# PhiFEM/phiFEM

Measured on NVIDIA B200. Metric: phi-FEM cells assembled/s (tags+CSR), higher is better.
Workload: dtype f64

## Files before the change

### include/phifem_b200.h

```cpp
#ifndef PHIFEM_B200_H
#define PHIFEM_B200_H

#include <stdint.h>

#ifdef __cplusplus
extern "C" {
#endif

#define PHIFEM_B200_ABI_VERSION 1

typedef enum phifem_status {
  PHIFEM_OK = 0,
  PHIFEM_ERR_ARGUMENT = -1,
  PHIFEM_ERR_CUDA = -2,
  PHIFEM_ERR_UNSUPPORTED = -3
} phifem_status;

typedef enum phifem_cell_type {
  PHIFEM_TRIANGLE = 0,
  PHIFEM_QUADRILATERAL = 1,
  PHIFEM_TETRAHEDRON = 2
} phifem_cell_type;

typedef struct phifem_mesh {
// ... 108 lines not shown
  const int16_t* seg_start;
  const int32_t* seg_dest;
  int64_t n_cell_inst;
  const int32_t* cell_verts;
  const int16_t* cell_pos;
  int64_t n_ghost_inst;
  const int32_t* ghost_facet;
  const int16_t* ghost_pos;
  int64_t n_bnd_inst;
  const int32_t* bnd_entity;
  const int16_t* bnd_pos;
} phifem_blocked_plan;

int phifem_assemble_blocked_p1(const phifem_mesh* mesh, const double* phi, const double* f, double sigma,
                               const phifem_blocked_plan* plan, double* data, double* b, void* stream);

typedef struct phifem_row_list {
  int64_t n_listed;
  const int32_t* rows;
  const uint8_t* diag_pos;
  const int32_t* ptr;
  const uint32_t* rec;
} phifem_row_list;

typedef struct phifem_cell_tiles {
  int32_t rows_per_tile;
  int32_t n_tiles;
  int64_t n_listed;
  const int32_t* rows;
  const uint8_t* diag_pos;
  const int32_t* chunk_ptr;
  const int32_t* slot_verts;
  const int32_t* rec_base;
  const uint16_t* rec_off;
  const uint32_t* rec;
  const uint32_t* push;
} phifem_cell_tiles;

typedef struct phifem_rows_plan {
  const int32_t* indptr;
  const int32_t* indices;
  int32_t max_row_nnz;
  int32_t reserved;
  phifem_row_list cells;
  phifem_row_list surface;
  int64_t n_ghost_facets;
  const int32_t* ghost_macro;
  int64_t n_entities;
  const int32_t* entity_macro;
  double* surface_work;
  const double* cell_geom;
  const phifem_cell_tiles* tiles;
  double* surface_static;
} phifem_rows_plan;

int phifem_assemble_rows_p1(const phifem_mesh* mesh, const double* phi, const double* f, double sigma,
                            const phifem_rows_plan* plan, double* data, double* b, void* stream);

typedef struct phifem_pk_space {
  int32_t degree;
  int32_t n_dofs_per_cell;
  int64_t n_dofs;
  const int32_t* dofmap;
} phifem_pk_space;

typedef struct phifem_quadrature {
  int32_t n_cell_points;
  int32_t n_facet_points;
  const double* cell_points;
  const double* cell_weights;
  const double* facet_points;
  const double* facet_weights;
} phifem_quadrature;

int phifem_assemble_cells_pk(const phifem_mesh* mesh, const phifem_pk_space* space_w,
                             const phifem_pk_space* space_phi, const phifem_quadrature* quad,
                             const double* phi, const double* f, const int8_t* cell_tags8,
                             const int32_t* active, int64_t n_active, const int32_t* slots, double sigma,
                             double* data, double* b, void* stream);

int phifem_assemble_boundary_pk(const phifem_mesh* mesh, const phifem_pk_space* space_w,
                                const phifem_pk_space* space_phi, const phifem_quadrature* quad,
                                const double* phi, const int32_t* entities, int64_t n_entities,
                                const int32_t* slots, double* data, void* stream);

int phifem_assemble_ghost_pk(const phifem_mesh* mesh, const phifem_pk_space* space_w,
                             const phifem_pk_space* space_phi, const phifem_quadrature* quad,
                             const double* phi, const int32_t* facets, int64_t n_facets,
                             const int32_t* slots, double sigma, double* data, void* stream);

int phifem_assemble_weak_cells_pk(const phifem_mesh* mesh, const phifem_pk_space* space_w,
                                  const phifem_pk_space* space_phi, const phifem_quadrature* quad,
                                  const double* phi, const double* f, const double* u_d,
                                  const int8_t* cell_tags8, const int32_t* active, int64_t n_active,
                                  const int32_t* slots, const int32_t* mixed_dofmap, double gamma,
                                  double sigma, double* data, double* b, void* stream);

int phifem_assemble_weak_boundary_pk(const phifem_mesh* mesh, const phifem_pk_space* space_w,
                                     const phifem_quadrature* quad, const int32_t* entities,
                                     int64_t n_entities, const int32_t* slots, double* data, void* stream);

int phifem_assemble_weak_ghost_pk(const phifem_mesh* mesh, const phifem_pk_space* space_w,
                                  const phifem_quadrature* quad, const int32_t* facets, int64_t n_facets,
                                  const int32_t* slots, double sigma, double* data, void* stream);

int phifem_csr_spmv(int64_t n_rows, const int32_t* indptr, const int32_t* indices, const double* data,
// ... 114 lines not shown
```

### phifem_b200/_lib.py

```python
import ctypes
import os

import torch

_HERE = os.path.dirname(os.path.abspath(__file__))
LIB_PATH = os.environ.get("PHIFEM_B200_LIB") or os.path.join(_HERE, "libphifem_b200.so")

CELL_TYPE_ID = {"triangle": 0, "quadrilateral": 1, "tetrahedron": 2}
N_COUNTERS = 16
CNT_INTERIOR, CNT_CUT, CNT_EXTERIOR, CNT_UNTAGGED, CNT_ZERO_DEN, CNT_ZERO_DEN_AMBIGUOUS = 0, 1, 2, 3, 4, 5
CNT_FACET_ZERO_DEN, CNT_FACET_CONFLICT, CNT_BOUNDARY_OWNERS = 11, 12, 13
CNT_CALLER0, CNT_CALLER1 = 14, 15

_vp = ctypes.c_void_p


class CMesh(ctypes.Structure):
    _fields_ = [("cell_type", ctypes.c_int32), ("gdim", ctypes.c_int32),
                ("n_vertices", ctypes.c_int64), ("n_cells", ctypes.c_int64),
                ("n_facets", ctypes.c_int64),
                ("x", _vp), ("cells", _vp), ("c2f", _vp), ("f2c", _vp),
                ("detj_min", ctypes.c_double), ("detj_max", ctypes.c_double),
                ("boundary_facets", _vp), ("n_boundary_facets", ctypes.c_int64),
                ("boundary_owner", _vp), ("boundary_scale", _vp), ("x4", _vp)]


class CLevelset(ctypes.Structure):
    _fields_ = [("mode", ctypes.c_int32), ("n_dofs_per_cell", ctypes.c_int32),
                ("n_cell_points", ctypes.c_int32), ("n_facet_points", ctypes.c_int32),
                ("coeffs", _vp), ("dofmap", _vp), ("cell_table", _vp), ("facet_table", _vp),
                ("cell_values", _vp), ("facet_values", _vp), ("coord_grad", _vp)]


class CBlockedPlan(ctypes.Structure):
    _fields_ = [("n_blocks", ctypes.c_int32), ("capacity", ctypes.c_int32),
                ("max_segments", ctypes.c_int32), ("reserved", ctypes.c_int32),
                ("block_desc", _vp), ("seg_start", _vp), ("seg_dest", _vp),
                ("n_cell_inst", ctypes.c_int64), ("cell_verts", _vp), ("cell_pos", _vp),
                ("n_ghost_inst", ctypes.c_int64), ("ghost_facet", _vp), ("ghost_pos", _vp),
                ("n_bnd_inst", ctypes.c_int64), ("bnd_entity", _vp), ("bnd_pos", _vp)]


class CRowList(ctypes.Structure):
    _fields_ = [("n_listed", ctypes.c_int64), ("rows", _vp), ("diag_pos", _vp), ("ptr", _vp), ("rec", _vp)]


class CCellTiles(ctypes.Structure):
    _fields_ = [("rows_per_tile", ctypes.c_int32), ("n_tiles", ctypes.c_int32), ("n_listed", ctypes.c_int64),
                ("rows", _vp), ("diag_pos", _vp), ("chunk_ptr", _vp), ("slot_verts", _vp), ("rec_base", _vp),
                ("rec_off", _vp), ("rec", _vp), ("push", _vp)]


class CRowsPlan(ctypes.Structure):
    _fields_ = [("indptr", _vp), ("indices", _vp), ("max_row_nnz", ctypes.c_int32),
                ("reserved", ctypes.c_int32), ("cells", CRowList), ("surface", CRowList),
                ("n_ghost_facets", ctypes.c_int64), ("ghost_macro", _vp), ("n_entities", ctypes.c_int64),
                ("entity_macro", _vp), ("surface_work", _vp), ("cell_geom", _vp),
                ("tiles", ctypes.POINTER(CCellTiles)), ("surface_static", _vp)]


class CRowsPlanInfo(ctypes.Structure):
    _fields_ = [("n_rows", ctypes.c_int64), ("nnz", ctypes.c_int64), ("n_active", ctypes.c_int64),
                ("n_ghost", ctypes.c_int64), ("n_entities", ctypes.c_int64), ("active", _vp), ("ghost", _vp),
                ("n_cell_records", ctypes.c_int64), ("n_surface_records", ctypes.c_int64),
                ("cells_record_slots", ctypes.c_int64), ("surface_record_slots", ctypes.c_int64)]


class CPkSpace(ctypes.Structure):
    _fields_ = [("degree", ctypes.c_int32), ("n_dofs_per_cell", ctypes.c_int32), ("n_dofs", ctypes.c_int64),
                ("dofmap", _vp)]


class CQuadrature(ctypes.Structure):
    _fields_ = [("n_cell_points", ctypes.c_int32), ("n_facet_points", ctypes.c_int32),
                ("cell_points", _vp), ("cell_weights", _vp), ("facet_points", _vp), ("facet_weights", _vp)]


class CPatternView(ctypes.Structure):
    _fields_ = [("n_rows", ctypes.c_int64), ("nnz", ctypes.c_int64), ("n_active", ctypes.c_int64),
                ("n_ghost", ctypes.c_int64), ("n_entities", ctypes.c_int64), ("indptr", _vp), ("indices", _vp),
                ("active", _vp), ("ghost", _vp), ("slots_cells", _vp), ("slots_ghost", _vp), ("slots_boundary", _vp)]


class CElasticityParams(ctypes.Structure):
    _fields_ = [(n, ctypes.c_double) for n in ("lmbda_in", "mu_in", "lmbda_out", "mu_out", "coef_in", "coef_out",
                                               "gamma", "sigma_s")]


_PK_HEAD = [ctypes.POINTER(CMesh), ctypes.POINTER(CPkSpace), ctypes.POINTER(CPkSpace),
            ctypes.POINTER(CQuadrature)]

_SIGNATURES = {
    "phifem_last_error": (ctypes.c_char_p, []),
    "phifem_abi_version": (ctypes.c_int, []),
    "phifem_post_to_host": (ctypes.c_int, [_vp, _vp, ctypes.c_int32, _vp]),
    "phifem_tags_match": (ctypes.c_int, [_vp, _vp, ctypes.c_int64, _vp, _vp, ctypes.c_int64, _vp, _vp]),
    "phifem_cell_points": (ctypes.c_int, [ctypes.POINTER(CMesh), _vp, ctypes.c_int32, _vp, _vp]),
    "phifem_tag_cells": (ctypes.c_int, [ctypes.POINTER(CMesh), ctypes.POINTER(CLevelset),
                                        ctypes.c_int32, _vp, _vp, _vp, _vp, _vp]),
    "phifem_tag_facets": (ctypes.c_int, [ctypes.POINTER(CMesh), ctypes.POINTER(CLevelset), _vp, _vp,
                                         _vp, _vp, _vp]),
    "phifem_boundary_records": (ctypes.c_int, [ctypes.POINTER(CMesh), _vp, _vp, _vp]),
    "phifem_tag_facets_phase": (ctypes.c_int, [ctypes.POINTER(CMesh), ctypes.POINTER(CLevelset), _vp, _vp,
                                               _vp, _vp, ctypes.c_int32, _vp]),
    "phifem_entity_records": (ctypes.c_int, [ctypes.POINTER(CMesh), _vp, _vp, ctypes.c_int32,
                                             ctypes.c_uint32, _vp, ctypes.c_int64, _vp, _vp]),
    "phifem_assemble_cells_p1": (ctypes.c_int, [ctypes.POINTER(CMesh), _vp, _vp, _vp, _vp,
                                                ctypes.c_int64, _vp, ctypes.c_double, _vp, _vp, _vp]),
    "phifem_assemble_boundary_p1": (ctypes.c_int, [ctypes.POINTER(CMesh), _vp, _vp, ctypes.c_int64,
                                                   _vp, _vp, _vp]),
    "phifem_assemble_ghost_p1": (ctypes.c_int, [ctypes.POINTER(CMesh), _vp, _vp, ctypes.c_int64, _vp,
# ... 156 lines not shown
```

### phifem_b200/assemble.py

```python
import numpy as np
import torch

from . import _lib
from .fem import Function
from .mesh import Measure


class CSRMatrix:

    def __init__(self, indptr, indices, data, shape):
        self.indptr, self.indices, self.data, self.shape = indptr, indices, data, shape

    def to_scipy(self):
        import scipy.sparse as sp
        return sp.csr_matrix((self.data.cpu().numpy(), self.indices.cpu().numpy(),
                              self.indptr.cpu().numpy()), shape=self.shape)


def ghost_macro_vertices(mesh, facets):
    g = facets.long()
    nv = mesh.cells.shape[1]
    out = []
    for side in (0, 1):
        c = mesh.f2c[g, side].long()
        cv = mesh.cells[c].long()
        lf = (mesh.c2f[c].long() == g[:, None]).long().argmax(dim=1)
        if side == 0:
            keep = torch.arange(nv, device=g.device)[None, :] != lf[:, None]
            out.append(cv[keep].reshape(-1, nv - 1))
        out.append(cv.gather(1, lf[:, None]))
    return torch.cat(out, dim=1)


class AssemblyPlan:

    def __init__(self, mesh, cell_tags8, facet_tags8, entities, method="rows", capacity=None,
                 order="auto", row_mask=None, geometry=False, cell_pass="rows", rows_per_tile=256, symbolic="auto"):
        if mesh.cell_type not in ("triangle", "tetrahedron"):
            raise NotImplementedError("P1 assembly supports triangles and tetrahedra")
        dev = mesh.device
        self.mesh = mesh
        self.cell_tags8 = cell_tags8
        self._sig_cells = cell_tags8.clone()
        self._sig_facets = _facet_classes(facet_tags8)
        n = mesh.num_vertices
        nv = mesh.cells.shape[1]
        self.n_rows = n
        ents2 = entities.reshape(-1, 2)
        if ents2.shape[0]:
            t = cell_tags8[ents2[:, 0].long()]
            if not bool(((t == 1) | (t == 2)).all()):
                raise ValueError("a (cell, local facet) entity names a cell that is not tagged 1 or 2: the strong-/weak-"
                                 "Dirichlet plans take the entities of ds(100) (Gamma_h seen from Omega_h)")
        if symbolic not in ("auto", "torch", "native"):
            raise ValueError("symbolic must be 'auto', 'torch' or 'native'")
        native_ok = (method == "rows" and cell_pass == "rows" and not geometry and dev.type == "cuda")
        if symbolic == "native" and not native_ok:
            raise ValueError("the native symbolic phase builds row-gather plans (method='rows', cell_pass='rows') on "
                             "CUDA meshes")
        self._slots = None
        if native_ok and symbolic in ("auto", "native"):
            from . import rows as rows_mod
            try:
                if order == "auto":
                    order = "natural"
                rp = rows_mod.NativeRowsPlan(mesh, cell_tags8, facet_tags8, entities, order=order, row_mask=row_mask)
            except NotImplementedError:
                if symbolic == "native":
                    raise
                rp = None
            if rp is not None:
                self.entities = entities.reshape(-1, 2).to(torch.int32).contiguous()
                self.active, self.ghost, self.indptr, self.indices, self.nnz = rp.active, rp.ghost, rp.indptr, \
                    rp.indices, rp.nnz
                self.blocked, self.rowsplan, self.method, self.symbolic = None, rp, "rows", "native"
                return
        self.symbolic = "torch"
        self.active = torch.nonzero((cell_tags8 == 1) | (cell_tags8 == 2)).reshape(-1).to(torch.int32)
        interior = mesh.f2c[:, 1] >= 0
        self.ghost = torch.nonzero(((facet_tags8 == 2) | (facet_tags8 == 3)) & interior) \
            .reshape(-1).to(torch.int32)
        self.entities = entities.reshape(-1, 2).to(torch.int32).contiguous()

        def pair_keys(dm):
            return (dm[:, :, None] * n + dm[:, None, :]).reshape(dm.shape[0], dm.shape[1] * dm.shape[1])

        dm = mesh.cells[self.active.long()].long()
        keys_c = pair_keys(dm)
        mac = ghost_macro_vertices(mesh, self.ghost)
        keys_g = pair_keys(mac)
        n_c = keys_c.numel()
        uniq, inv = torch.unique(torch.cat([keys_c.reshape(-1), keys_g.reshape(-1)]), sorted=True,
                                 return_inverse=True)
        del keys_c, keys_g
        slots_cells = inv[:n_c].reshape(-1, nv * nv).to(torch.int32).contiguous()
        slots_ghost = inv[n_c:].reshape(-1, (nv + 1) ** 2).to(torch.int32).contiguous()
        del inv
        keys_b = pair_keys(mesh.cells[self.entities[:, 0].long()].long())
        slots_boundary = torch.searchsorted(uniq, keys_b.reshape(-1)).reshape(-1, nv * nv) \
            .to(torch.int32).contiguous()
        self._slots = (slots_cells, slots_ghost, slots_boundary)
        rows = uniq // n
        self.indices = (uniq - rows * n).to(torch.int32).contiguous()
        counts = torch.bincount(rows, minlength=n)
        self.indptr = torch.zeros(n + 1, dtype=torch.int64, device=dev)
        self.indptr[1:] = torch.cumsum(counts, dim=0)
        self.indptr = self.indptr.to(torch.int32).contiguous()
        self.nnz = int(uniq.numel())
        if self.nnz >= 2 ** 31:
            raise NotImplementedError("CSR pattern with %d entries: indptr / slot maps are int32 (PETSc's default "
                                      "index width too); shard the mesh (phifem_b200/partition.py)" % self.nnz)
        self.blocked, self.rowsplan, self.method = None, None, "atomic"
        if method == "rows" and self.nnz > 0:
            from . import rows as rows_mod
            try:
                self.rowsplan = rows_mod.RowsPlan(self, order=order, row_mask=row_mask, geometry=geometry,
                                                  cell_pass=cell_pass, rows_per_tile=rows_per_tile)
                self.method = "rows"
            except NotImplementedError:
                self.rowsplan = None
        elif method == "blocked" and self.active.numel() > 0:
            from . import blocked
            try:
                self.blocked = blocked.BlockedPlan(self, capacity or blocked.DEFAULT_CAPACITY)
                self.method = "blocked"
            except NotImplementedError:
                self.blocked = None
        elif method not in ("rows", "blocked", "atomic"):
            raise ValueError("method must be 'rows', 'blocked' or 'atomic'")

    def _slot_maps(self):
        if self._slots is None:
            n, nv = self.n_rows, self.mesh.cells.shape[1]
            ip = self.indptr.long()
            rows = torch.repeat_interleave(torch.arange(n, device=self.mesh.device), ip[1:] - ip[:-1])
            keys = rows * n + self.indices.long()
            del rows

            def slots(dm):
                k = (dm[:, :, None] * n + dm[:, None, :]).reshape(-1)
                return torch.searchsorted(keys, k).reshape(dm.shape[0], -1).to(torch.int32).contiguous()
            cells = self.mesh.cells
            self._slots = (slots(cells[self.active.long()].long()), slots(ghost_macro_vertices(self.mesh, self.ghost)),
                           slots(cells[self.entities[:, 0].long()].long()))
        return self._slots

    slots_cells = property(lambda self: self._slot_maps()[0])
    slots_ghost = property(lambda self: self._slot_maps()[1])
    slots_boundary = property(lambda self: self._slot_maps()[2])

    def new_outputs(self):
        dev = self.mesh.device
        return (torch.zeros(self.nnz, dtype=torch.float64, device=dev),
                torch.zeros(self.n_rows, dtype=torch.float64, device=dev))

    def matches(self, cells_tags, facets_tags):
        c8, f8, _ = _plan_inputs(self.mesh, cells_tags, facets_tags, None)
        if c8.numel() != self._sig_cells.numel() or f8.numel() != self._sig_facets.numel():
            return False
        if c8.is_cuda:
            bad = torch.empty(1, dtype=torch.int64, device=c8.device)
            _lib.check(_lib.load().phifem_tags_match(_lib.ptr(c8), _lib.ptr(self._sig_cells), c8.numel(), _lib.ptr(f8),
                                                     _lib.ptr(self._sig_facets), f8.numel(), _lib.ptr(bad), _lib.stream()))
            return int(bad.item()) == 0
        return bool(torch.equal(c8, self._sig_cells)) and bool(torch.equal(_facet_classes(f8), self._sig_facets))


def _facet_classes(facet_tags8):
    return ((facet_tags8 == 2) | (facet_tags8 == 3)).to(torch.int8) + 2 * (facet_tags8 == 4).to(torch.int8)


def _plan_inputs(mesh, cells_tags, facets_tags, ds):
    from .mesh_scripts import _narrow_tags
    c8 = getattr(cells_tags, "tags8", None)
    c8 = c8 if c8 is not None else _narrow_tags(cells_tags.values_dev)
    f8 = getattr(facets_tags, "tags8", None)
    f8 = f8 if f8 is not None else _narrow_tags(facets_tags.values_dev)
    if ds is None:
        ents = torch.zeros(0, dtype=torch.int32, device=mesh.device)
    elif isinstance(ds, Measure) and ds.subdomain_data is None:
        bf = mesh.boundary_facets.long()
        owner = mesh.f2c[bf, 0].long()
        lf = (mesh.c2f[owner].long() == bf[:, None]).long().argmax(dim=1)
        ents = torch.stack([owner, lf], dim=1).reshape(-1).to(torch.int32)
    elif hasattr(ds, "integration_entities_dev"):
        ents = ds.integration_entities_dev
    elif torch.is_tensor(ds):
        ents = ds.to(mesh.device)
    else:
        ents = torch.as_tensor(np.asarray(ds, dtype=np.int32), device=mesh.device)
    return c8.contiguous(), f8.contiguous(), ents


def build_plan(mesh, cells_tags, facets_tags, ds=None, method="rows", capacity=None, order="auto",
               V=None, V_phi=None, geometry=False, cell_pass="rows", rows_per_tile=256, symbolic="auto"):
    c8, f8, ents = _plan_inputs(mesh, cells_tags, facets_tags, ds)
    if mesh.cell_type == "quadrilateral":
        if method not in ("rows", "pk"):
            raise ValueError("method=%r: quadrilateral meshes are assembled by the quadrature kernels only" % method)
        if geometry or cell_pass != "rows" or symbolic == "native":
            raise ValueError("geometry, cell_pass and symbolic='native' are options of the row-gather plans, which "
                             "have no quadrilateral implementation")
        from . import fem
        from .assemble_pk import PkAssemblyPlan
        V = fem.functionspace(mesh, 1) if V is None else V
        V_phi = V if V_phi is None else V_phi
        return PkAssemblyPlan(mesh, c8, f8, ents, V, V_phi)
    V_phi = V if V_phi is None else V_phi
    V = V_phi if V is None else V
    if V is not None and (V.degree != 1 or V_phi.degree != 1 or method == "pk"):
        from .assemble_pk import PkAssemblyPlan
        return PkAssemblyPlan(mesh, c8, f8, ents, V, V_phi)
    return AssemblyPlan(mesh, c8, f8, ents, method=method, capacity=capacity,
                        order=order, geometry=geometry, cell_pass=cell_pass, rows_per_tile=rows_per_tile,
                        symbolic=symbolic)


def _device_vector(mesh, v, space=None):
    if isinstance(v, Function):
        if space is None and v.function_space.degree != 1:
            raise NotImplementedError("this plan was built for P1 (vertex dofs); pass V / V_phi to build_plan")
        if space is not None and v.function_space.degree != space.degree:
            raise ValueError("coefficient of degree %d given where the plan expects degree %d"
                             % (v.function_space.degree, space.degree))
        v = v.x.array
    t = v if torch.is_tensor(v) else torch.from_numpy(np.ascontiguousarray(v, dtype=np.float64))
    t = t.to(mesh.device, dtype=torch.float64, non_blocking=True).contiguous()
    n = mesh.num_vertices if space is None else space.num_dofs
    if t.numel() != n:
        raise ValueError("expected %d dof values, got %d" % (n, t.numel()))
    return t


def assemble_into(plan, phi, f, sigma, data, b, marks=None):
    if getattr(plan, "V", None) is not None:
        from .assemble_pk import assemble_pk_into
        return assemble_pk_into(plan, phi, f, sigma, data, b, marks=marks)
    marks_given = marks is not None
    marks = marks or (lambda: None)
    _lib.require_cuda(plan.mesh)
    if getattr(plan, "rowsplan", None) is not None:
        from . import rows as rows_mod
        marks()
        if marks_given:
            rows_mod.assemble_rows_into(plan.rowsplan, phi, f, sigma, data, b, passes=("cells",))
            marks()
            marks()
            rows_mod.assemble_rows_into(plan.rowsplan, phi, f, sigma, data, b, passes=("surface",))
            marks()
        else:
            rows_mod.assemble_rows_into(plan.rowsplan, phi, f, sigma, data, b)
        return data, b
    if getattr(plan, "blocked", None) is not None:
        from . import blocked
        marks()
        blocked.assemble_blocked_into(plan.blocked, phi, f, sigma, data, b)
        marks()
        marks()
        marks()
        return data, b
    lib = _lib.load()
    cm = _lib.c_mesh(plan.mesh)
    st = _lib.stream()
    data.zero_()
    b.zero_()
    marks()
    _lib.check(lib.phifem_assemble_cells_p1(
        cm, _lib.ptr(phi), _lib.ptr(f), _lib.ptr(plan.cell_tags8), _lib.ptr(plan.active),
# ... 75 lines not shown
```

### phifem_b200/csrc/assemble_rows.cu

```cuda
#include <stdlib.h>

#include <type_traits>

#include "common.cuh"
#include "p1_forms.cuh"

namespace phifem {
namespace {

#ifndef PHIFEM_ROWS_BLOCK
#define PHIFEM_ROWS_BLOCK 64
#endif
constexpr int kRowsBlock = PHIFEM_ROWS_BLOCK;
#ifndef PHIFEM_ROWS_MINBLOCKS
#define PHIFEM_ROWS_MINBLOCKS (512 / PHIFEM_ROWS_BLOCK)
#endif
#ifndef PHIFEM_SURF_MINBLOCKS
#define PHIFEM_SURF_MINBLOCKS PHIFEM_ROWS_MINBLOCKS
#endif
#ifndef PHIFEM_SURF_DEPTH
#define PHIFEM_SURF_DEPTH 2
#endif
#ifndef PHIFEM_ONCE_MINBLOCKS
#define PHIFEM_ONCE_MINBLOCKS 1
// ... 632 lines not shown
  if constexpr (KIND != kSurface) {
    for (int k = 0; k < nnz; ++k) data[start + k] = acc[k * kRowsBlock];
    b[r] = br;
  } else {
    for (int k = 0; k < nnz; ++k) data[start + k] += acc[k * kRowsBlock];
  }
}

}
}

using namespace phifem;

namespace phifem {
cudaError_t launch_cell_tiles_p1(const phifem_mesh* mesh, const double* phi, const double* f, double sigma,
                                 const int32_t* indptr, const phifem_cell_tiles* tl, int max_row_nnz, double* data,
                                 double* b, cudaStream_t st);
}

namespace {
bool list_ok(const phifem_row_list& l) {
  return l.n_listed == 0 || (l.rows && l.diag_pos && l.ptr && l.rec);
}
struct SideStream {
  cudaStream_t stream = nullptr;
  cudaEvent_t fork = nullptr, join = nullptr;
  bool ok = false;
};
SideStream& side_stream() {
  static SideStream per_device[64];
  int dev = 0;
  cudaGetDevice(&dev);
  SideStream& s = per_device[dev & 63];
  if (!s.stream) {
    s.ok = cudaStreamCreateWithFlags(&s.stream, cudaStreamNonBlocking) == cudaSuccess &&
           cudaEventCreateWithFlags(&s.fork, cudaEventDisableTiming) == cudaSuccess &&
           cudaEventCreateWithFlags(&s.join, cudaEventDisableTiming) == cudaSuccess;
  }
  return s;
}
}

extern "C" int phifem_assemble_rows_p1(const phifem_mesh* mesh, const double* phi, const double* f,
                                       double sigma, const phifem_rows_plan* plan, double* data,
                                       double* b, void* stream) {
  PHIFEM_CHECK_ARG(mesh != nullptr && mesh->x, "mesh is null");
  if (mesh->cell_type != PHIFEM_TRIANGLE && mesh->cell_type != PHIFEM_TETRAHEDRON) {
    set_error("P1 assembly supports triangles and tetrahedra, got cell type %d", mesh->cell_type);
    return PHIFEM_ERR_UNSUPPORTED;
  }
  PHIFEM_CHECK_ARG(mesh->gdim == (mesh->cell_type == PHIFEM_TRIANGLE ? 2 : 3), "gdim mismatch");
  PHIFEM_CHECK_ARG(plan != nullptr, "plan is null");
  const phifem_cell_tiles* tiles = plan->tiles && plan->tiles->n_tiles > 0 ? plan->tiles : nullptr;
  if (plan->cells.n_listed == 0 && plan->surface.n_listed == 0 && !tiles) return PHIFEM_OK;
  PHIFEM_CHECK_ARG(phi && f && data && b, "null pointer");
  PHIFEM_CHECK_ARG(plan->indptr && plan->indices, "CSR pattern is null");
  PHIFEM_CHECK_ARG(list_ok(plan->cells) && list_ok(plan->surface), "row list arrays are null");
  PHIFEM_CHECK_ARG(plan->max_row_nnz > 0 && plan->max_row_nnz <= 255, "plan.max_row_nnz out of range");
  const int64_t n_once = plan->surface.n_listed ? plan->n_ghost_facets + plan->n_entities : 0;
  PHIFEM_CHECK_ARG(plan->surface.n_listed == 0 ||
                       (n_once > 0 && n_once < (1 << 28) && plan->surface_work &&
                        (plan->n_ghost_facets == 0 || plan->ghost_macro) &&
                        (plan->n_entities == 0 || plan->entity_macro)),
                   "surface arrays (n_ghost_facets + n_entities < 2^28, ghost_macro, entity_macro, surface_work)");
  const size_t smem = (size_t)plan->max_row_nnz * kRowsBlock * sizeof(double);
  cudaStream_t st = (cudaStream_t)stream;
  cudaError_t err = cudaSuccess;
  auto launch = [&](auto kernel, const phifem_row_list& rl, const double* work, const double* coords = nullptr) {
    if (rl.n_listed == 0 || err != cudaSuccess) return;
    if (smem > 48 * 1024)
      err = cudaFuncSetAttribute(kernel, cudaFuncAttributeMaxDynamicSharedMemorySize, (int)smem);
    const int64_t grid = (rl.n_listed + kRowsBlock - 1) / kRowsBlock;
    if (err == cudaSuccess)
      kernel<<<(unsigned)grid, kRowsBlock, smem, st>>>(coords ? coords : mesh->x, phi, f, sigma, plan->indptr,
                                                       plan->indices, rl, work, data, b);
  };
  const bool use_x4 = mesh->x4 != nullptr;
  const bool geom = plan->cell_geom != nullptr;
  auto cell_tiles = [&]() {
    if (err == cudaSuccess)
      err = launch_cell_tiles_p1(mesh, phi, f, sigma, plan->indptr, tiles, plan->max_row_nnz, data, b, st);
  };
  SideStream& ss = side_stream();
  const bool fork = n_once > 0 && (plan->cells.n_listed > 0 || tiles) && ss.ok;
  cudaStream_t once_stream = fork ? ss.stream : st;
  auto once = [&](auto dim) {
    constexpr int D = decltype(dim)::value;
    if (n_once == 0) return;
    if (fork) {
      cudaEventRecord(ss.fork, st);
      cudaStreamWaitEvent(ss.stream, ss.fork, 0);
    }
    const unsigned grid = (unsigned)((n_once + kRowsBlock - 1) / kRowsBlock);
    if (plan->surface_static)
      k_surface_fill_p1<D><<<grid, kRowsBlock, 0, once_stream>>>(phi, sigma, plan->ghost_macro, plan->n_ghost_facets,
                                                                 plan->entity_macro, plan->n_entities,
                                                                 plan->surface_static, plan->surface_work);
    else
      k_surface_once_p1<D><<<grid, kRowsBlock, 0, once_stream>>>(mesh->x, phi, sigma, plan->ghost_macro,
                                                                 plan->n_ghost_facets, plan->entity_macro,
                                                                 plan->n_entities, plan->surface_work);
    if (fork) cudaEventRecord(ss.join, ss.stream);
  };
  if (mesh->cell_type == PHIFEM_TRIANGLE) {
    once(std::integral_constant<int, 2>());
    if (tiles) cell_tiles();
    else if (geom) launch(k_assemble_rows_p1<2, kCellsGeom>, plan->cells, plan->cell_geom);
    else launch(k_assemble_rows_p1<2, kCells>, plan->cells, nullptr);
    if (fork) cudaStreamWaitEvent(st, ss.join, 0);
    launch(k_assemble_rows_p1<2, kSurface>, plan->surface, plan->surface_work);
  } else {
    once(std::integral_constant<int, 3>());
    if (tiles) cell_tiles();
    else if (geom) launch(k_assemble_rows_p1<3, kCellsGeom>, plan->cells, plan->cell_geom);
    else if (use_x4) launch(k_assemble_rows_p1<3, kCellsX4>, plan->cells, nullptr, mesh->x4);
    else launch(k_assemble_rows_p1<3, kCells>, plan->cells, nullptr);
    if (fork) cudaStreamWaitEvent(st, ss.join, 0);
    launch(k_assemble_rows_p1<3, kSurface>, plan->surface, plan->surface_work);
  }
  if (err != cudaSuccess) {
    set_error("phifem_assemble_rows_p1: launch failed (%zu bytes of shared memory per row-gather CTA%s): %s", smem,
              tiles ? ", cell tiles" : "", cudaGetErrorString(err));
    return PHIFEM_ERR_CUDA;
  }
  PHIFEM_CHECK_LAUNCH();
  return PHIFEM_OK;
}

extern "C" int phifem_surface_static_p1(const phifem_mesh* mesh, const phifem_rows_plan* plan, void* stream) {
  PHIFEM_CHECK_ARG(mesh != nullptr && mesh->x && plan != nullptr, "mesh / plan is null");
  if (mesh->cell_type != PHIFEM_TRIANGLE && mesh->cell_type != PHIFEM_TETRAHEDRON) {
    set_error("P1 assembly supports triangles and tetrahedra, got cell type %d", mesh->cell_type);
    return PHIFEM_ERR_UNSUPPORTED;
  }
  const int64_t n_once = plan->n_ghost_facets + plan->n_entities;
  if (n_once == 0) return PHIFEM_OK;
  PHIFEM_CHECK_ARG(plan->surface_static != nullptr, "plan.surface_static is null");
  PHIFEM_CHECK_ARG((plan->n_ghost_facets == 0 || plan->ghost_macro) && (plan->n_entities == 0 || plan->entity_macro),
                   "ghost_macro / entity_macro");
  cudaStream_t st = (cudaStream_t)stream;
  const unsigned grid = (unsigned)((n_once + kRowsBlock - 1) / kRowsBlock);
  if (mesh->cell_type == PHIFEM_TRIANGLE)
    k_surface_static_p1<2><<<grid, kRowsBlock, 0, st>>>(mesh->x, plan->ghost_macro, plan->n_ghost_facets,
                                                        plan->entity_macro, plan->n_entities, plan->surface_static);
  else
    k_surface_static_p1<3><<<grid, kRowsBlock, 0, st>>>(mesh->x, plan->ghost_macro, plan->n_ghost_facets,
                                                        plan->entity_macro, plan->n_entities, plan->surface_static);
  PHIFEM_CHECK_LAUNCH();
  return PHIFEM_OK;
}
```

### phifem_b200/rows.py

```python
import ctypes

import torch

from . import _lib

PAD = 0xFFFFFFFF
MAX_ROW_NNZ = 255
MAX_SMEM_BYTES = 200 * 1024
BLOCK = 128
BALANCE_CHUNK = 4096


def morton_order(x, rows):
    from .mesh import morton_keys
    return rows[torch.argsort(morton_keys(x[rows]), stable=True)]


class RowList:

    def __init__(self, rows, diag_slot, indptr, rec_rows, words, n_rows, balance=False):
        dev = rows.device
        i64 = dict(dtype=torch.int64, device=dev)
        if balance and rows.numel():
            per_row = torch.bincount(rec_rows, minlength=n_rows)[rows]
            chunk = torch.arange(rows.numel(), **i64) // BALANCE_CHUNK
            key = chunk * (int(per_row.max()) + 1) + (int(per_row.max()) - per_row)
            rows = rows[torch.argsort(key, stable=True)]
        self.n_listed = int(rows.numel())
        self.n_slices = (self.n_listed + 31) // 32
        self.words = w = words.shape[1]
        self.n_records = int(rec_rows.numel())
        self.rows = rows.to(torch.int32).contiguous()
        self.diag_pos = (diag_slot[rows] - indptr[rows]).to(torch.uint8).contiguous()
        ns = self.n_slices
        li_of_row = torch.full((n_rows,), -1, **i64)
        li_of_row[rows] = torch.arange(self.n_listed, **i64)
        li = li_of_row[rec_rows]
        assert self.n_records == 0 or int(li.min()) >= 0, "a record names a row outside its list"
        counts = torch.bincount(li, minlength=ns * 32)[:ns * 32]
        width = counts.reshape(ns, 32).max(dim=1).values if ns else torch.zeros(0, **i64)
        ptr = torch.zeros(ns + 1, **i64)
        ptr[1:] = torch.cumsum(width, 0)
        total = int(ptr[-1])
        if total * 32 * w >= 2 ** 31:
            raise NotImplementedError("row-gather plan: record array exceeds 2^31 words")
        rec = torch.full((max(total, 1) * 32, w), PAD, **i64)
        if self.n_records:
            order = torch.argsort(li, stable=True)
            ls = li[order]
            first = torch.cumsum(counts, 0) - counts
            k = torch.arange(ls.numel(), **i64) - first[ls]
            rec[(ptr[ls >> 5] + k) * 32 + (ls & 31)] = words[order]
        rec = rec.reshape(-1)
        rec = torch.where(rec >= 2 ** 31, rec - 2 ** 32, rec).to(torch.int32)
        self.ptr, self.rec = ptr.to(torch.int32).contiguous(), rec.contiguous()

    def c_struct(self):
        p = _lib.ptr
        return _lib.CRowList(self.n_listed, p(self.rows), p(self.diag_pos), p(self.ptr), p(self.rec))

    def nbytes(self):
        return int(sum(t.numel() * t.element_size() for t in (self.rows, self.diag_pos, self.ptr, self.rec)))

    def padding(self):
        return 1.0 - self.n_records * self.words / max(1, self.rec.numel())


def _pack_bytes(pos):
    word = torch.zeros(pos.shape[0], dtype=torch.int64, device=pos.device)
    for j in range(pos.shape[1]):
        word |= pos[:, j] << (8 * j)
    return word


def cell_geometry(x, cells):
    n, nv = cells.shape
    d = nv - 1
    X = x[cells.long()]
    e = X[:, 1:, :] - X[:, :1, :]
    if d == 2:
        R = [None, torch.stack([e[:, 1, 1], -e[:, 1, 0]], dim=1), torch.stack([-e[:, 0, 1], e[:, 0, 0]], dim=1)]
        det = e[:, 0, 0] * e[:, 1, 1] - e[:, 1, 0] * e[:, 0, 1]
        dfact = 2.0
    else:
        def cross(a, b):
            return torch.stack([a[:, 1] * b[:, 2] - a[:, 2] * b[:, 1], a[:, 2] * b[:, 0] - a[:, 0] * b[:, 2],
                                a[:, 0] * b[:, 1] - a[:, 1] * b[:, 0]], dim=1)
        R = [None, cross(e[:, 1], e[:, 2]), cross(e[:, 2], e[:, 0]), cross(e[:, 0], e[:, 1])]
        det = e[:, 0, 0] * R[1][:, 0] + e[:, 0, 1] * R[1][:, 1] + e[:, 0, 2] * R[1][:, 2]
        dfact = 6.0
    R[0] = -(R[1] + R[2]) if d == 2 else -(R[1] + R[2] + R[3])
    out = torch.zeros((n, 8), dtype=torch.float64, device=x.device)
    scale = 1.0 / (dfact * det.abs())
    k = 0
    for a in range(nv):
        for b in range(a + 1, nv):
            out[:, k] = (R[a] * R[b]).sum(dim=1) * scale
            k += 1
    out[:, k] = det.abs() / dfact
    h2 = torch.zeros(n, dtype=torch.float64, device=x.device)
    for a in range(nv):
        for b in range(a + 1, nv):
            h2 = torch.maximum(h2, ((X[:, a] - X[:, b]) ** 2).sum(dim=1))
    out[:, k + 1] = h2
    return out.contiguous()


class RowsPlan:

    def __init__(self, plan, order="natural", row_mask=None, geometry=False, cell_pass="rows", rows_per_tile=256):
        mesh = plan.mesh
        dev = mesh.device
        d = mesh.gdim
        nv = d + 1
        n = plan.n_rows
        i64 = dict(dtype=torch.int64, device=dev)
        self.plan = plan
        indptr = plan.indptr.long()
        row_nnz = indptr[1:] - indptr[:-1]
        has = row_nnz > 0
        if row_mask is not None:
            has = has & row_mask.to(dev)
        listed = torch.nonzero(has).reshape(-1)
        self.max_row_nnz = int(row_nnz[listed].max()) if listed.numel() else 0

        def owned(rec_rows, words):
            if row_mask is None or rec_rows.numel() == 0:
                return rec_rows, words
            keep = row_mask.to(dev)[rec_rows]
            return rec_rows[keep], words[keep]

        if self.max_row_nnz > MAX_ROW_NNZ or self.max_row_nnz * BLOCK * 8 > MAX_SMEM_BYTES:
            raise NotImplementedError(
                "row-gather assembly: a row holds %d entries (limit %d); use the atomic scatter kernels "
                "for this mesh" % (self.max_row_nnz, min(MAX_ROW_NNZ, MAX_SMEM_BYTES // (BLOCK * 8))))
        if order not in ("natural", "morton", "auto"):
            raise ValueError("order must be 'natural', 'morton' or 'auto'")
        if cell_pass not in ("rows", "tiles", "push"):
            raise ValueError("cell_pass must be 'rows', 'tiles' or 'push'")
        if cell_pass in ("tiles", "push") and (geometry or self.max_row_nnz > 128):
            cell_pass = "rows"
        if order == "auto":
            order = "morton" if cell_pass in ("tiles", "push") and not getattr(mesh, "sfc_ordered", False) else "natural"
        self.order = order
        self.cell_pass = cell_pass

        def ordered(rows):
            rows = torch.unique(rows)
            return morton_order(mesh.x, rows) if order == "morton" and rows.numel() else rows

        def surface_ordered(rows):
            rows = torch.unique(rows)
            return morton_order(mesh.x, rows) if rows.numel() else rows

        cols = plan.indices.long()
        row_of_slot = torch.repeat_interleave(torch.arange(n, **i64), row_nnz)
        is_diag = cols == row_of_slot
        dslot = torch.full((n,), -1, **i64)
        dslot[row_of_slot[is_diag]] = torch.nonzero(is_diag).reshape(-1)
        assert bool((dslot[listed] >= 0).all()), "a listed row has no diagonal entry"
        del row_of_slot, is_diag, cols

        cells_act = mesh.cells[plan.active.long()].long()
# ... 27 lines not shown
        ng = int(plan.ghost.numel())
        if ng:
            mac = ghost_macro_vertices(mesh, plan.ghost)
            gs = plan.slots_ghost.long().reshape(-1, nv + 1, nv + 1)
            if ng >= 2 ** 28:
                raise NotImplementedError("row-gather plan: more than 2^28 ghost-penalty facets")
            words = []
            gidx = torch.arange(ng, **i64)
            for a in range(nv + 1):
                others = [j for j in range(nv + 1) if j != a]
                pos = gs[:, a, others] - indptr[mac[:, a]][:, None]
                words.append(torch.stack([_pack_bytes(pos), gidx | (a << 28)], dim=1))
            rec_rows, words = mac.reshape(-1), torch.stack(words, dim=1).reshape(-1, 2)
            self.ghost_macro = mac.to(torch.int32).contiguous()
        else:
            rec_rows, words = torch.zeros(0, **i64), torch.zeros((0, 2), **i64)
            self.ghost_macro = torch.zeros((0, nv + 1), dtype=torch.int32, device=dev)
        self.n_ghost_facets = ng
        ghost_rows, ghost_words = owned(rec_rows, words)

        ne = int(plan.entities.shape[0])
        self.n_entities = ne
        if ng + ne >= 2 ** 28:
            raise NotImplementedError("row-gather plan: more than 2^28 surface entities")
        if ne:
            ec = plan.entities[:, 0].long()
            eo = plan.entities[:, 1].long()
            ev = mesh.cells[ec].long()
            bs = plan.slots_boundary.long().reshape(-1, nv, nv)
            ar = torch.arange(ne, **i64)
            loc = torch.arange(nv, **i64)[None, :].expand(ne, nv)
            fac = loc[loc != eo[:, None]].reshape(ne, d)
            rec_rows, words = [], []
            for t in range(d):
                i = fac[:, t]
                rest = fac[:, [(t + u) % d for u in range(1, d)]]
                oth = torch.cat([eo[:, None], rest], dim=1)
                row = ev[ar, i]
                pos = bs[ar[:, None], i[:, None], oth] - indptr[row][:, None]
                words.append(torch.stack([_pack_bytes(pos), (ng + ar) | (t << 28) | (1 << 31)], dim=1))
                rec_rows.append(row)
            rec_rows = torch.stack(rec_rows, dim=1).reshape(-1)
            words = torch.stack(words, dim=1).reshape(-1, 2)
            self.entity_macro = torch.cat([ev.gather(1, fac), ev.gather(1, eo[:, None])], dim=1) \
                .to(torch.int32).contiguous()
        else:
            rec_rows, words = torch.zeros(0, **i64), torch.zeros((0, 2), **i64)
            self.entity_macro = torch.zeros((0, nv), dtype=torch.int32, device=dev)
        ent_rows, ent_words = owned(rec_rows, words)
        rec_rows = torch.cat([ghost_rows, ent_rows])
        words = torch.cat([ghost_words, ent_words])
        self.n_ghost_records, self.n_entity_records = int(ghost_rows.numel()), int(ent_rows.numel())
        self.surface = RowList(surface_ordered(rec_rows), dslot, indptr, rec_rows, words, n, balance=True)
        self.surface_work = torch.empty((max(ng + ne, 1), 8), dtype=torch.float64, device=dev)
        self.surface_static = torch.zeros((max(ng + ne, 1), 8), dtype=torch.float64, device=dev) if dev.type == "cuda" \
            else None
        self._c = None
        if self.surface_static is not None and ng + ne > 0:
            _lib.check(_lib.load().phifem_surface_static_p1(_lib.c_mesh(mesh), ctypes.byref(self.c_struct()),
                                                            _lib.stream()))

    def c_struct(self, passes=None):
        if passes is not None:
            p = _lib.ptr
            empty = _lib.CRowList(0, None, None, None, None)
            lists = [getattr(self, nm).c_struct() if nm in passes else empty for nm in ("cells", "surface")]
            return _lib.CRowsPlan(p(self.plan.indptr), p(self.plan.indices), self.max_row_nnz, 0, *lists,
                                  *self._surface_fields(cells="cells" in passes))
        if self._c is None:
            p = _lib.ptr
            pl = self.plan
            self._c = _lib.CRowsPlan(p(pl.indptr), p(pl.indices), self.max_row_nnz, 0,
                                     self.cells.c_struct(), self.surface.c_struct(), *self._surface_fields())
        return self._c

    def _surface_fields(self, cells=True):
        if self.surface_work.device.type != "cuda":
            return 0, None, 0, None, None, None, None, None
        return (self.n_ghost_facets, _lib.ptr(self.ghost_macro) if self.n_ghost_facets else None,
                self.n_entities, _lib.ptr(self.entity_macro) if self.n_entities else None,
                _lib.ptr(self.surface_work), _lib.ptr(self.cell_geom),
                ctypes.pointer(self.tiles.c_struct()) if self.tiles is not None and cells else None,
                _lib.ptr(self.surface_static))

    def index_bytes(self):
        return (self.cells.nbytes() + (self.tiles.nbytes() if self.tiles is not None else 0)
                + self.surface.nbytes() + self.ghost_macro.numel() * 4
                + self.entity_macro.numel() * 4 + self.surface_work.numel() * 8
                + (self.surface_static.numel() * 8 if self.surface_static is not None else 0)
                + (self.cell_geom.numel() * 8 if self.cell_geom is not None else 0))


class _NativeList:

    def __init__(self, c_list, n_records, slots, words, device, keep):
        self.c = c_list
        self.n_listed = int(c_list.n_listed)
        self.n_slices = (self.n_listed + 31) // 32
        self.words, self.n_records, self._slots = words, int(n_records), int(slots)
        def dv(*a):
            return _lib.device_view(*a, owner=keep)
        self.rows = dv(c_list.rows, (self.n_listed,), torch.int32, device)
        self.diag_pos = dv(c_list.diag_pos, (self.n_listed,), torch.uint8, device)
        self.ptr = dv(c_list.ptr, (self.n_slices + 1,), torch.int32, device)
        self.rec = dv(c_list.rec, (max(self._slots, 32) * words,), torch.int32, device)
        self._keep = keep

    def c_struct(self):
        return self.c

    def nbytes(self):
        return self.n_listed * 5 + (self.n_slices + 1) * 4 + max(self._slots, 32) * self.words * 4

    def padding(self):
        return 1.0 - self.n_records / max(1, self._slots)


class _Handle:
    def __init__(self, pointer):
        self.pointer = pointer

    def __del__(self):
        try:
            if self.pointer:
                _lib.load().phifem_rows_plan_destroy(self.pointer)
        except Exception:
            pass
        self.pointer = None


class NativeRowsPlan:

    def __init__(self, mesh, cell_tags8, facet_tags8, entities, order="natural", row_mask=None):
        _lib.require_cuda(mesh)
        lib = _lib.load()
        dev = mesh.device
        ents = entities.reshape(-1, 2).to(torch.int32).contiguous()
        mask = None if row_mask is None else row_mask.to(dev).to(torch.uint8).contiguous()
        out = ctypes.c_void_p()
        _lib.check(lib.phifem_rows_plan_create(_lib.c_mesh(mesh), _lib.ptr(cell_tags8), _lib.ptr(facet_tags8),
                                               _lib.ptr(ents) if ents.numel() else None, ents.shape[0],
                                               _lib.ptr(mask), 1 if order == "morton" else 0, ctypes.byref(out),
                                               _lib.stream()))
        self._handle = _Handle(out.value)
        self._c, info = _lib.CRowsPlan(), _lib.CRowsPlanInfo()
        _lib.check(lib.phifem_rows_plan_view(out.value, ctypes.byref(self._c), ctypes.byref(info)))
        self.info = info
        self.mesh, self.order, self.cell_pass, self.tiles, self.cell_geom = mesh, order, "rows", None, None
        nv = mesh.cells.shape[1]

        def dv(*a):
            return _lib.device_view(*a, owner=self._handle)
        self.n_rows, self.nnz = int(info.n_rows), int(info.nnz)
        self.indptr = dv(self._c.indptr, (self.n_rows + 1,), torch.int32, dev)
        self.indices = dv(self._c.indices, (self.nnz,), torch.int32, dev)
        self.active = dv(info.active, (int(info.n_active),), torch.int32, dev)
        self.ghost = dv(info.ghost, (int(info.n_ghost),), torch.int32, dev)
        self.max_row_nnz = int(self._c.max_row_nnz)
        self.n_ghost_facets, self.n_entities = int(info.n_ghost), int(info.n_entities)
        self.ghost_macro = dv(self._c.ghost_macro, (self.n_ghost_facets, nv + 1), torch.int32, dev)
        self.entity_macro = dv(self._c.entity_macro, (self.n_entities, nv), torch.int32, dev)
        self.surface_work = dv(self._c.surface_work, (max(self.n_ghost_facets + self.n_entities, 1), 8), torch.float64,
                               dev)
        self.surface_static = dv(self._c.surface_static, (max(self.n_ghost_facets + self.n_entities, 1), 8),
                                 torch.float64, dev)
        n_cell_rec = int(info.n_cell_records)
        if mask is not None:
            cnt = (self.indptr[1:] > self.indptr[:-1]) & mask.bool()
            deg = torch.bincount(mesh.cells[self.active.long()].long().reshape(-1), minlength=self.n_rows)
            n_cell_rec = int(deg[cnt].sum())
        self.n_cell_records = n_cell_rec
        self.cells = _NativeList(self._c.cells, n_cell_rec, info.cells_record_slots, 1, dev, self._handle)
        self.surface = _NativeList(self._c.surface, info.n_surface_records, info.surface_record_slots, 2, dev,
                                   self._handle)
        self.n_ghost_records = self.n_ghost_facets * (nv + 1) if mask is None else None
        self.n_entity_records = self.n_entities * (nv - 1) if mask is None else None

    def c_struct(self, passes=None):
        if passes is None:
            return self._c
        c = _lib.CRowsPlan()
        ctypes.pointer(c)[0] = self._c
        empty = _lib.CRowList(0, None, None, None, None)
        if "cells" not in passes:
            c.cells = empty
        if "surface" not in passes:
            c.surface = empty
        return c

    def index_bytes(self):
        return (self.cells.nbytes() + self.surface.nbytes() + self.ghost_macro.numel() * 4
                + self.entity_macro.numel() * 4 + self.surface_work.numel() * 8 + self.surface_static.numel() * 8)


def assemble_rows_into(rplan, phi, f, sigma, data, b, passes=None):
    mesh = rplan.mesh if isinstance(rplan, NativeRowsPlan) else rplan.plan.mesh
    _lib.require_cuda(mesh)
    _lib.check(_lib.load().phifem_assemble_rows_p1(
        _lib.c_mesh(mesh), _lib.ptr(phi), _lib.ptr(f), float(sigma),
        ctypes.byref(rplan.c_struct(passes)), _lib.ptr(data), _lib.ptr(b), _lib.stream()))
    return data, b
```

Baseline: 28.81 billion.

## Reorder cell-pass rows so rows touched by surface pass run first

Builds an alternative cell row list in which rows near cut cells or surface records come first, in Morton order and load-balanced, followed by the remaining rows. The kernel uses this list when present, and it is on by default. The aim is for the surface pass, which runs after the cell pass and the side-stream join, to find the rows it shares with the cell pass still in cache, and possibly to overlap better with the side stream. In exchange it adds a second record array (more memory and plan-build time) and can lose the locality of the natural row order for interior rows.

```diff
diff --git a/include/phifem_b200.h b/include/phifem_b200.h
--- a/include/phifem_b200.h
+++ b/include/phifem_b200.h
@@ -184,6 +184,7 @@
   const double* cell_geom;
   const phifem_cell_tiles* tiles;
   double* surface_static;
+  phifem_row_list cells_surface_first;
 } phifem_rows_plan;
 
 int phifem_assemble_rows_p1(const phifem_mesh* mesh, const double* phi, const double* f, double sigma,
diff --git a/phifem_b200/_lib.py b/phifem_b200/_lib.py
--- a/phifem_b200/_lib.py
+++ b/phifem_b200/_lib.py
@@ -56,7 +56,8 @@
                 ("reserved", ctypes.c_int32), ("cells", CRowList), ("surface", CRowList),
                 ("n_ghost_facets", ctypes.c_int64), ("ghost_macro", _vp), ("n_entities", ctypes.c_int64),
                 ("entity_macro", _vp), ("surface_work", _vp), ("cell_geom", _vp),
-                ("tiles", ctypes.POINTER(CCellTiles)), ("surface_static", _vp)]
+                ("tiles", ctypes.POINTER(CCellTiles)), ("surface_static", _vp),
+                ("cells_surface_first", CRowList)]
 
 
 class CRowsPlanInfo(ctypes.Structure):
diff --git a/phifem_b200/assemble.py b/phifem_b200/assemble.py
--- a/phifem_b200/assemble.py
+++ b/phifem_b200/assemble.py
@@ -35,7 +35,8 @@
 class AssemblyPlan:
 
     def __init__(self, mesh, cell_tags8, facet_tags8, entities, method="rows", capacity=None,
-                 order="auto", row_mask=None, geometry=False, cell_pass="rows", rows_per_tile=256, symbolic="auto"):
+                 order="auto", row_mask=None, geometry=False, cell_pass="rows", rows_per_tile=256, symbolic="auto",
+                 surface_first=True):
         if mesh.cell_type not in ("triangle", "tetrahedron"):
             raise NotImplementedError("P1 assembly supports triangles and tetrahedra")
         dev = mesh.device
@@ -64,7 +65,8 @@
             try:
                 if order == "auto":
                     order = "natural"
-                rp = rows_mod.NativeRowsPlan(mesh, cell_tags8, facet_tags8, entities, order=order, row_mask=row_mask)
+                rp = rows_mod.NativeRowsPlan(mesh, cell_tags8, facet_tags8, entities, order=order, row_mask=row_mask,
+                                             surface_first=surface_first)
             except NotImplementedError:
                 if symbolic == "native":
                     raise
@@ -115,7 +117,8 @@
             from . import rows as rows_mod
             try:
                 self.rowsplan = rows_mod.RowsPlan(self, order=order, row_mask=row_mask, geometry=geometry,
-                                                  cell_pass=cell_pass, rows_per_tile=rows_per_tile)
+                                                  cell_pass=cell_pass, rows_per_tile=rows_per_tile,
+                                                  surface_first=surface_first)
                 self.method = "rows"
             except NotImplementedError:
                 self.rowsplan = None
@@ -193,7 +196,8 @@
 
 
 def build_plan(mesh, cells_tags, facets_tags, ds=None, method="rows", capacity=None, order="auto",
-               V=None, V_phi=None, geometry=False, cell_pass="rows", rows_per_tile=256, symbolic="auto"):
+               V=None, V_phi=None, geometry=False, cell_pass="rows", rows_per_tile=256, symbolic="auto",
+               surface_first=True):
     c8, f8, ents = _plan_inputs(mesh, cells_tags, facets_tags, ds)
     if mesh.cell_type == "quadrilateral":
         if method not in ("rows", "pk"):
@@ -213,7 +217,7 @@
         return PkAssemblyPlan(mesh, c8, f8, ents, V, V_phi)
     return AssemblyPlan(mesh, c8, f8, ents, method=method, capacity=capacity,
                         order=order, geometry=geometry, cell_pass=cell_pass, rows_per_tile=rows_per_tile,
-                        symbolic=symbolic)
+                        symbolic=symbolic, surface_first=surface_first)
 
 
 def _device_vector(mesh, v, space=None):
diff --git a/phifem_b200/csrc/assemble_rows.cu b/phifem_b200/csrc/assemble_rows.cu
--- a/phifem_b200/csrc/assemble_rows.cu
+++ b/phifem_b200/csrc/assemble_rows.cu
@@ -708,10 +708,11 @@
   PHIFEM_CHECK_ARG(mesh->gdim == (mesh->cell_type == PHIFEM_TRIANGLE ? 2 : 3), "gdim mismatch");
   PHIFEM_CHECK_ARG(plan != nullptr, "plan is null");
   const phifem_cell_tiles* tiles = plan->tiles && plan->tiles->n_tiles > 0 ? plan->tiles : nullptr;
-  if (plan->cells.n_listed == 0 && plan->surface.n_listed == 0 && !tiles) return PHIFEM_OK;
+  const phifem_row_list& cells = plan->cells_surface_first.n_listed ? plan->cells_surface_first : plan->cells;
+  if (cells.n_listed == 0 && plan->surface.n_listed == 0 && !tiles) return PHIFEM_OK;
   PHIFEM_CHECK_ARG(phi && f && data && b, "null pointer");
   PHIFEM_CHECK_ARG(plan->indptr && plan->indices, "CSR pattern is null");
-  PHIFEM_CHECK_ARG(list_ok(plan->cells) && list_ok(plan->surface), "row list arrays are null");
+  PHIFEM_CHECK_ARG(list_ok(cells) && list_ok(plan->surface), "row list arrays are null");
   PHIFEM_CHECK_ARG(plan->max_row_nnz > 0 && plan->max_row_nnz <= 255, "plan.max_row_nnz out of range");
   const int64_t n_once = plan->surface.n_listed ? plan->n_ghost_facets + plan->n_entities : 0;
   PHIFEM_CHECK_ARG(plan->surface.n_listed == 0 ||
@@ -738,7 +739,7 @@
       err = launch_cell_tiles_p1(mesh, phi, f, sigma, plan->indptr, tiles, plan->max_row_nnz, data, b, st);
   };
   SideStream& ss = side_stream();
-  const bool fork = n_once > 0 && (plan->cells.n_listed > 0 || tiles) && ss.ok;
+  const bool fork = n_once > 0 && (cells.n_listed > 0 || tiles) && ss.ok;
   cudaStream_t once_stream = fork ? ss.stream : st;
   auto once = [&](auto dim) {
     constexpr int D = decltype(dim)::value;
@@ -761,16 +762,16 @@
   if (mesh->cell_type == PHIFEM_TRIANGLE) {
     once(std::integral_constant<int, 2>());
     if (tiles) cell_tiles();
-    else if (geom) launch(k_assemble_rows_p1<2, kCellsGeom>, plan->cells, plan->cell_geom);
-    else launch(k_assemble_rows_p1<2, kCells>, plan->cells, nullptr);
+    else if (geom) launch(k_assemble_rows_p1<2, kCellsGeom>, cells, plan->cell_geom);
+    else launch(k_assemble_rows_p1<2, kCells>, cells, nullptr);
     if (fork) cudaStreamWaitEvent(st, ss.join, 0);
     launch(k_assemble_rows_p1<2, kSurface>, plan->surface, plan->surface_work);
   } else {
     once(std::integral_constant<int, 3>());
     if (tiles) cell_tiles();
-    else if (geom) launch(k_assemble_rows_p1<3, kCellsGeom>, plan->cells, plan->cell_geom);
-    else if (use_x4) launch(k_assemble_rows_p1<3, kCellsX4>, plan->cells, nullptr, mesh->x4);
-    else launch(k_assemble_rows_p1<3, kCells>, plan->cells, nullptr);
+    else if (geom) launch(k_assemble_rows_p1<3, kCellsGeom>, cells, plan->cell_geom);
+    else if (use_x4) launch(k_assemble_rows_p1<3, kCellsX4>, cells, nullptr, mesh->x4);
+    else launch(k_assemble_rows_p1<3, kCells>, cells, nullptr);
     if (fork) cudaStreamWaitEvent(st, ss.join, 0);
     launch(k_assemble_rows_p1<3, kSurface>, plan->surface, plan->surface_work);
   }
diff --git a/phifem_b200/rows.py b/phifem_b200/rows.py
--- a/phifem_b200/rows.py
+++ b/phifem_b200/rows.py
@@ -22,21 +22,33 @@
         dev = rows.device
         i64 = dict(dtype=torch.int64, device=dev)
         if balance and rows.numel():
-            per_row = torch.bincount(rec_rows, minlength=n_rows)[rows]
-            chunk = torch.arange(rows.numel(), **i64) // BALANCE_CHUNK
-            key = chunk * (int(per_row.max()) + 1) + (int(per_row.max()) - per_row)
-            rows = rows[torch.argsort(key, stable=True)]
+            rows = _balanced(rows, torch.bincount(rec_rows, minlength=n_rows)[rows])
+        li_of_row = torch.full((n_rows,), -1, **i64)
+        li_of_row[rows] = torch.arange(rows.numel(), **i64)
+        li = li_of_row[rec_rows]
+        assert li.numel() == 0 or int(li.min()) >= 0, "a record names a row outside its list"
+        order = torch.argsort(li, stable=True)
+        ls = li[order]
+        counts = torch.bincount(ls, minlength=rows.numel())
+        first = torch.cumsum(counts, 0) - counts
+        k = torch.arange(ls.numel(), **i64) - first[ls]
+        self._fill(rows, diag_slot[rows] - indptr[rows], ls, k, words[order])
+
+    @classmethod
+    def from_ranked(cls, rows, diag_pos, li, k, words):
+        self = cls.__new__(cls)
+        self._fill(rows, diag_pos, li, k, words)
+        return self
+
+    def _fill(self, rows, diag_pos, li, k, words):
+        i64 = dict(dtype=torch.int64, device=rows.device)
         self.n_listed = int(rows.numel())
         self.n_slices = (self.n_listed + 31) // 32
         self.words = w = words.shape[1]
-        self.n_records = int(rec_rows.numel())
+        self.n_records = int(li.numel())
         self.rows = rows.to(torch.int32).contiguous()
-        self.diag_pos = (diag_slot[rows] - indptr[rows]).to(torch.uint8).contiguous()
+        self.diag_pos = diag_pos.to(torch.uint8).contiguous()
         ns = self.n_slices
-        li_of_row = torch.full((n_rows,), -1, **i64)
-        li_of_row[rows] = torch.arange(self.n_listed, **i64)
-        li = li_of_row[rec_rows]
-        assert self.n_records == 0 or int(li.min()) >= 0, "a record names a row outside its list"
         counts = torch.bincount(li, minlength=ns * 32)[:ns * 32]
         width = counts.reshape(ns, 32).max(dim=1).values if ns else torch.zeros(0, **i64)
         ptr = torch.zeros(ns + 1, **i64)
@@ -46,11 +58,7 @@
             raise NotImplementedError("row-gather plan: record array exceeds 2^31 words")
         rec = torch.full((max(total, 1) * 32, w), PAD, **i64)
         if self.n_records:
-            order = torch.argsort(li, stable=True)
-            ls = li[order]
-            first = torch.cumsum(counts, 0) - counts
-            k = torch.arange(ls.numel(), **i64) - first[ls]
-            rec[(ptr[ls >> 5] + k) * 32 + (ls & 31)] = words[order]
+            rec[(ptr[li >> 5] + k) * 32 + (li & 31)] = words
         rec = rec.reshape(-1)
         rec = torch.where(rec >= 2 ** 31, rec - 2 ** 32, rec).to(torch.int32)
         self.ptr, self.rec = ptr.to(torch.int32).contiguous(), rec.contiguous()
@@ -64,6 +72,47 @@
 
     def padding(self):
         return 1.0 - self.n_records * self.words / max(1, self.rec.numel())
+
+
+def _balanced(rows, weight):
+    chunk = torch.arange(rows.numel(), dtype=torch.int64, device=rows.device) // BALANCE_CHUNK
+    top = int(weight.max())
+    return rows[torch.argsort(chunk * (top + 1) + (top - weight), stable=True)]
+
+
+def _records(rl):
+    dev = rl.rows.device
+    i64 = dict(dtype=torch.int64, device=dev)
+    w = rl.words
+    total = int(rl.ptr[-1]) if rl.n_listed else 0
+    if total == 0:
+        return torch.zeros(0, **i64), torch.zeros(0, **i64), torch.zeros((0, w), **i64)
+    ptr = rl.ptr.long()
+    slice_of = torch.repeat_interleave(torch.arange(rl.n_slices, **i64), ptr[1:] - ptr[:-1], output_size=total)
+    k = (torch.arange(total, **i64) - ptr[slice_of])[:, None].expand(total, 32)
+    li = slice_of[:, None] * 32 + torch.arange(32, **i64)
+    words = rl.rec[:total * 32 * w].reshape(total, 32, w).long() & 0xFFFFFFFF
+    real = words[:, :, w - 1] != PAD
+    return li[real], k[real], words[real]
+
+
+def surface_rows_first(x, cells, surface, n_rows):
+    dev = cells.rows.device
+    i64 = dict(dtype=torch.int64, device=dev)
+    c_li, c_k, c_w = _records(cells)
+    crows = cells.rows.long()
+    near = torch.zeros(n_rows, dtype=torch.bool, device=dev)
+    near[crows[c_li[((c_w[:, 0] >> 24) & 1) == 1]]] = True
+    near[surface.rows.long()] = True
+    first = torch.nonzero(near).reshape(-1)
+    if first.numel():
+        first = _balanced(morton_order(x, first), torch.bincount(crows[c_li], minlength=n_rows)[first])
+    rows = torch.cat([first, crows[~near[crows]]])
+    li_of_row = torch.full((n_rows,), -1, **i64)
+    li_of_row[rows] = torch.arange(rows.numel(), **i64)
+    diag = torch.zeros(n_rows, dtype=torch.uint8, device=dev)
+    diag[crows] = cells.diag_pos
+    return RowList.from_ranked(rows, diag[rows], li_of_row[crows[c_li]], c_k, c_w)
 
 
 def _pack_bytes(pos):
@@ -108,7 +157,8 @@
 
 class RowsPlan:
 
-    def __init__(self, plan, order="natural", row_mask=None, geometry=False, cell_pass="rows", rows_per_tile=256):
+    def __init__(self, plan, order="natural", row_mask=None, geometry=False, cell_pass="rows", rows_per_tile=256,
+                 surface_first=True):
         mesh = plan.mesh
         dev = mesh.device
         d = mesh.gdim
@@ -242,6 +292,9 @@
         words = torch.cat([ghost_words, ent_words])
         self.n_ghost_records, self.n_entity_records = int(ghost_rows.numel()), int(ent_rows.numel())
         self.surface = RowList(surface_ordered(rec_rows), dslot, indptr, rec_rows, words, n, balance=True)
+        self.cells_surface_first = None
+        if surface_first and self.cell_pass == "rows" and not geometry:
+            self.cells_surface_first = surface_rows_first(mesh.x, self.cells, self.surface, n)
         self.surface_work = torch.empty((max(ng + ne, 1), 8), dtype=torch.float64, device=dev)
         self.surface_static = torch.zeros((max(ng + ne, 1), 8), dtype=torch.float64, device=dev) if dev.type == "cuda" \
             else None
@@ -256,12 +309,14 @@
             empty = _lib.CRowList(0, None, None, None, None)
             lists = [getattr(self, nm).c_struct() if nm in passes else empty for nm in ("cells", "surface")]
             return _lib.CRowsPlan(p(self.plan.indptr), p(self.plan.indices), self.max_row_nnz, 0, *lists,
-                                  *self._surface_fields(cells="cells" in passes))
+                                  *self._surface_fields(cells="cells" in passes),
+                                  _surface_first_field(self.cells_surface_first, passes))
         if self._c is None:
             p = _lib.ptr
             pl = self.plan
             self._c = _lib.CRowsPlan(p(pl.indptr), p(pl.indices), self.max_row_nnz, 0,
-                                     self.cells.c_struct(), self.surface.c_struct(), *self._surface_fields())
+                                     self.cells.c_struct(), self.surface.c_struct(), *self._surface_fields(),
+                                     _surface_first_field(self.cells_surface_first))
         return self._c
 
     def _surface_fields(self, cells=True):
@@ -278,7 +333,14 @@
                 + self.surface.nbytes() + self.ghost_macro.numel() * 4
                 + self.entity_macro.numel() * 4 + self.surface_work.numel() * 8
                 + (self.surface_static.numel() * 8 if self.surface_static is not None else 0)
-                + (self.cell_geom.numel() * 8 if self.cell_geom is not None else 0))
+                + (self.cell_geom.numel() * 8 if self.cell_geom is not None else 0)
+                + (self.cells_surface_first.nbytes() if self.cells_surface_first is not None else 0))
+
+
+def _surface_first_field(rl, passes=None):
+    if rl is None or (passes is not None and "cells" not in passes):
+        return _lib.CRowList(0, None, None, None, None)
+    return rl.c_struct()
 
 
 class _NativeList:
@@ -321,7 +383,7 @@
 
 class NativeRowsPlan:
 
-    def __init__(self, mesh, cell_tags8, facet_tags8, entities, order="natural", row_mask=None):
+    def __init__(self, mesh, cell_tags8, facet_tags8, entities, order="natural", row_mask=None, surface_first=True):
         _lib.require_cuda(mesh)
         lib = _lib.load()
         dev = mesh.device
@@ -365,6 +427,9 @@
                                    self._handle)
         self.n_ghost_records = self.n_ghost_facets * (nv + 1) if mask is None else None
         self.n_entity_records = self.n_entities * (nv - 1) if mask is None else None
+        self.cells_surface_first = surface_rows_first(mesh.x, self.cells, self.surface, self.n_rows) \
+            if surface_first else None
+        self._c.cells_surface_first = _surface_first_field(self.cells_surface_first)
 
     def c_struct(self, passes=None):
         if passes is None:
@@ -376,11 +441,13 @@
             c.cells = empty
         if "surface" not in passes:
             c.surface = empty
+        c.cells_surface_first = _surface_first_field(self.cells_surface_first, passes)
         return c
 
     def index_bytes(self):
         return (self.cells.nbytes() + self.surface.nbytes() + self.ghost_macro.numel() * 4
-                + self.entity_macro.numel() * 4 + self.surface_work.numel() * 8 + self.surface_static.numel() * 8)
+                + self.entity_macro.numel() * 4 + self.surface_work.numel() * 8 + self.surface_static.numel() * 8
+                + (self.cells_surface_first.nbytes() if self.cells_surface_first is not None else 0))
 
 
 def assemble_rows_into(rplan, phi, f, sigma, data, b, passes=None):
```

Result: slower. 27.61 billion (median of 6 runs) (-4.2%).
